# RobotLocomotion/pytorch-dense-correspondence

Measured on NVIDIA H100. Metric: image-pairs/s (640x480, D=3) fwd+loss+bwd, higher is better.
Workload: dtype f32 (bf16x3 split on the wgmma tensor cores, fp32 accumulate)

## Files before the change

pytorch-dense-correspondence_b200/csrc/conv_tc.cu:

```cuda
#include <cuda.h>
#include <algorithm>
#include <cstring>
#include <functional>
#include <mutex>
#include <unordered_map>

#include "conv.cuh"
#include "conv_tc.cuh"

namespace ddn {

constexpr int TC_BLOCK_K = 64;
constexpr int TC_CONSUMERS = 256;
constexpr int TC_THREADS = TC_CONSUMERS + 32;
constexpr int TC_PRODUCER_WARP = TC_CONSUMERS / 32;
constexpr int TC_WIDE_THREADS = TC_CONSUMERS + 128;
constexpr int TC_A_BYTES = 128 * TC_BLOCK_K * 2;

__device__ __forceinline__ uint32_t smem_u32(const void* p) { return (uint32_t)__cvta_generic_to_shared(p); }

__device__ __forceinline__ void mbar_init(uint32_t bar, uint32_t count) {
  asm volatile("mbarrier.init.shared::cta.b64 [%0], %1;" ::"r"(bar), "r"(count));
}
__device__ __forceinline__ void mbar_expect_tx(uint32_t bar, uint32_t bytes) {
// ... 110 lines not shown
  if (NPROD == 3) {
    Wgmma<N>::template mma<TRANS>(d, a_hi, b_lo, accumulate);
    Wgmma<N>::template mma<TRANS>(d, a_lo, b_hi, 1);
    Wgmma<N>::template mma<TRANS>(d, a_hi, b_hi, 1);
  } else {
    Wgmma<N>::template mma<TRANS>(d, a_hi, b_hi, accumulate);
  }
}
template <int N, int TRANS, int NPROD>
__device__ __forceinline__ void mma_k16_x(float (&d)[N / 2], float (&x)[N / 2], uint64_t a_hi, uint64_t a_lo, uint64_t b_hi, uint64_t b_lo,
                                          int accumulate) {
  if (NPROD == 3) {
    Wgmma<N>::template mma<TRANS>(x, a_hi, b_lo, accumulate);
    Wgmma<N>::template mma<TRANS>(x, a_lo, b_hi, 1);
  }
  Wgmma<N>::template mma<TRANS>(d, a_hi, b_hi, accumulate);
}
template <int K>
__device__ __forceinline__ void add_cross(float (&d)[K], const float (&x)[K]) {
#pragma unroll
  for (int i = 0; i < K; ++i) d[i] += x[i];
}
template <int N, int K>
__device__ __forceinline__ float (&acc_cols(float (&d)[K]))[N / 2] {
  static_assert(N / 2 <= K, "accumulator too narrow");
  return *reinterpret_cast<float(*)[N / 2]>(&d[0]);
}

constexpr int EPI_ROWS = 4;
constexpr int EPI_STRIDE = 40;
constexpr int EPI_WARP_FLOATS = 16 * EPI_STRIDE;

template <int K>
__device__ __forceinline__ void stage_write(const float (&acc)[K], int c, float* st, int lane) {
  const int r = lane >> 2, q = (lane & 3) * 2;
#pragma unroll
  for (int jj = 0; jj < 4; ++jj) {
    const int j = 4 * c + jj;
    *reinterpret_cast<float2*>(st + r * EPI_STRIDE + 8 * jj + q) = make_float2(acc[4 * j], acc[4 * j + 1]);
    *reinterpret_cast<float2*>(st + (r + 8) * EPI_STRIDE + 8 * jj + q) = make_float2(acc[4 * j + 2], acc[4 * j + 3]);
  }
  __syncwarp();
}

template <int K>
__device__ __forceinline__ void stage_chunk(const float (&acc)[K], int c, float* st, int lane, float4 (&v)[EPI_ROWS]) {
  stage_write(acc, c, st, lane);
  const int ga = lane >> 3, gb = lane & 7;
#pragma unroll
  for (int i = 0; i < EPI_ROWS; ++i) v[i] = *reinterpret_cast<const float4*>(st + (EPI_ROWS * ga + i) * EPI_STRIDE + 4 * gb);
  __syncwarp();
}

__device__ __forceinline__ uint32_t pack_bf16x2(__nv_bfloat16 a, __nv_bfloat16 b) {
  return (uint32_t)__bfloat16_as_ushort(a) | ((uint32_t)__bfloat16_as_ushort(b) << 16);
}

struct TcEpilogueParams {
  float* out;
  const float* addend;
  int imgs_per_group;
  BnFwdFinal fin;
  TcBwdStats bst;
  const float* ep_scale; const float* ep_shift; int ep_relu;
  __nv_bfloat16* out_hi; __nv_bfloat16* out_lo;
};

__device__ __forceinline__ void conv_epilogue_rows(const TcEpilogueParams& p, const float4 (&v)[EPI_ROWS], size_t off, size_t rs, int n_ok, int ch,
                                                   int C, int grp, float4& s1, float4& s2) {
  float4 adv[EPI_ROWS];
#pragma unroll
  for (int i = 0; i < EPI_ROWS; ++i)
    adv[i] = (p.addend && i < n_ok) ? __ldg(reinterpret_cast<const float4*>(p.addend + off + i * rs)) : make_float4(0.f, 0.f, 0.f, 0.f);
  if (p.ep_scale) {
    const float4 sc = __ldg(reinterpret_cast<const float4*>(p.ep_scale + ch));
    const float4 sh = __ldg(reinterpret_cast<const float4*>(p.ep_shift + ch));
#pragma unroll
    for (int i = 0; i < EPI_ROWS; ++i) {
      float4 f = make_float4(fmaf(v[i].x, sc.x, sh.x) + adv[i].x, fmaf(v[i].y, sc.y, sh.y) + adv[i].y,
                             fmaf(v[i].z, sc.z, sh.z) + adv[i].z, fmaf(v[i].w, sc.w, sh.w) + adv[i].w);
      if (p.ep_relu) { f.x = fmaxf(f.x, 0.f); f.y = fmaxf(f.y, 0.f); f.z = fmaxf(f.z, 0.f); f.w = fmaxf(f.w, 0.f); }
      if (i < n_ok) {
        if (p.out) *reinterpret_cast<float4*>(p.out + off + i * rs) = f;
        if (p.out_hi) {
          const __nv_bfloat16 h0 = __float2bfloat16_rn(f.x), h1 = __float2bfloat16_rn(f.y), h2 = __float2bfloat16_rn(f.z), h3 = __float2bfloat16_rn(f.w);
          *reinterpret_cast<uint2*>(p.out_hi + off + i * rs) = make_uint2(pack_bf16x2(h0, h1), pack_bf16x2(h2, h3));
          if (p.out_lo)
            *reinterpret_cast<uint2*>(p.out_lo + off + i * rs) =
                make_uint2(pack_bf16x2(__float2bfloat16_rn(f.x - __bfloat162float(h0)), __float2bfloat16_rn(f.y - __bfloat162float(h1))),
                           pack_bf16x2(__float2bfloat16_rn(f.z - __bfloat162float(h2)), __float2bfloat16_rn(f.w - __bfloat162float(h3))));
        }
      }
    }
  } else if (p.bst.fin.a.acc) {
    float4 rw[EPI_ROWS];
    uint2 yh[EPI_ROWS];
#pragma unroll
    for (int i = 0; i < EPI_ROWS; ++i) {
      rw[i] = i < n_ok ? __ldg(reinterpret_cast<const float4*>(p.bst.raw + off + i * rs)) : make_float4(0.f, 0.f, 0.f, 0.f);
      if (p.bst.y_hi) yh[i] = i < n_ok ? __ldg(reinterpret_cast<const uint2*>(p.bst.y_hi + off + i * rs)) : make_uint2(0u, 0u);
    }
    const float4 mu = __ldg(reinterpret_cast<const float4*>(p.bst.mean + (size_t)grp * C + ch));
    const float4 is = __ldg(reinterpret_cast<const float4*>(p.bst.invstd + (size_t)grp * C + ch));
    float4 scl = make_float4(0.f, 0.f, 0.f, 0.f), be = scl;
    if (!p.bst.y_hi && p.bst.relu) {
      const float4 gm = __ldg(reinterpret_cast<const float4*>(p.bst.gamma + ch));
      be = __ldg(reinterpret_cast<const float4*>(p.bst.beta + ch));
      scl = make_float4(gm.x * is.x, gm.y * is.y, gm.z * is.z, gm.w * is.w);
    }
#pragma unroll
    for (int i = 0; i < EPI_ROWS; ++i) {
      float4 g = make_float4(v[i].x + adv[i].x, v[i].y + adv[i].y, v[i].z + adv[i].z, v[i].w + adv[i].w);
      if (i < n_ok) *reinterpret_cast<float4*>(p.out + off + i * rs) = g;
      else g = make_float4(0.f, 0.f, 0.f, 0.f);
      if (p.bst.y_hi) {
        const uint2 hh = yh[i];
        if ((hh.x & 0x8000u) || !(hh.x & 0x7fffu)) g.x = 0.f;
        if ((hh.x & 0x80000000u) || !(hh.x & 0x7fff0000u)) g.y = 0.f;
        if ((hh.y & 0x8000u) || !(hh.y & 0x7fffu)) g.z = 0.f;
        if ((hh.y & 0x80000000u) || !(hh.y & 0x7fff0000u)) g.w = 0.f;
      } else if (p.bst.relu) {
        if (!(fmaf(rw[i].x - mu.x, scl.x, be.x) > 0.f)) g.x = 0.f;
        if (!(fmaf(rw[i].y - mu.y, scl.y, be.y) > 0.f)) g.y = 0.f;
        if (!(fmaf(rw[i].z - mu.z, scl.z, be.z) > 0.f)) g.z = 0.f;
        if (!(fmaf(rw[i].w - mu.w, scl.w, be.w) > 0.f)) g.w = 0.f;
      }
      s1.x += g.x; s1.y += g.y; s1.z += g.z; s1.w += g.w;
      s2.x = fmaf(g.x, (rw[i].x - mu.x) * is.x, s2.x); s2.y = fmaf(g.y, (rw[i].y - mu.y) * is.y, s2.y);
      s2.z = fmaf(g.z, (rw[i].z - mu.z) * is.z, s2.z); s2.w = fmaf(g.w, (rw[i].w - mu.w) * is.w, s2.w);
    }
  } else {
#pragma unroll
    for (int i = 0; i < EPI_ROWS; ++i) {
      const float4 raw = i < n_ok ? v[i] : make_float4(0.f, 0.f, 0.f, 0.f);
      if (i < n_ok)
        *reinterpret_cast<float4*>(p.out + off + i * rs) = make_float4(raw.x + adv[i].x, raw.y + adv[i].y, raw.z + adv[i].z, raw.w + adv[i].w);
      s1.x += raw.x; s1.y += raw.y; s1.z += raw.z; s1.w += raw.w;
      s2.x = fmaf(raw.x, raw.x, s2.x); s2.y = fmaf(raw.y, raw.y, s2.y); s2.z = fmaf(raw.z, raw.z, s2.z); s2.w = fmaf(raw.w, raw.w, s2.w);
    }
  }
}

__device__ __forceinline__ void colsum_lane_groups(float4& s1, float4& s2) {
#pragma unroll
  for (int off = 8; off < 32; off <<= 1) {
    s1.x += __shfl_xor_sync(0xffffffffu, s1.x, off); s1.y += __shfl_xor_sync(0xffffffffu, s1.y, off);
    s1.z += __shfl_xor_sync(0xffffffffu, s1.z, off); s1.w += __shfl_xor_sync(0xffffffffu, s1.w, off);
    s2.x += __shfl_xor_sync(0xffffffffu, s2.x, off); s2.y += __shfl_xor_sync(0xffffffffu, s2.y, off);
    s2.z += __shfl_xor_sync(0xffffffffu, s2.z, off); s2.w += __shfl_xor_sync(0xffffffffu, s2.w, off);
  }
}

__device__ __forceinline__ void named_barrier(int id, int threads) { asm volatile("bar.sync %0, %1;" ::"r"(id), "r"(threads) : "memory"); }
// ... 30 lines not shown
    const int j = idx - p.full_items;
    tile = p.full_items + j / p.tail_split;
    piece = j - (j / p.tail_split) * p.tail_split;
    width = block_n / p.tail_split;
  }
  TcItem it;
  it.sp = tile / p.n_co;
  it.co0 = (tile - it.sp * p.n_co) * block_n + piece * width;
  it.width = width;
  return it;
}
struct TcSub { int n, h0, w0; bool valid; };
__device__ __forceinline__ TcSub tc_sub(const TcConvParams& p, int st) {
  TcSub s;
  s.valid = st < p.n_sub;
  const int tw = st % p.tiles_w; const int t = st / p.tiles_w;
  const int th = t % p.tiles_h;
  s.n = s.valid ? t / p.tiles_h : p.N;
  s.h0 = th * TC_SUB_H; s.w0 = tw * TC_SUB_W;
  return s;
}

template <int W, int BLOCK_N, int NPROD, int STAGES, int TRANS = 0>
__device__ __forceinline__ void conv_tc_mainloop(float (&acc)[W / 2], float (&accx)[W / 2], int num_kb, uint32_t& g, const uint64_t* full_bar,
                                                 const uint64_t* empty_bar, const uint8_t* smem, int wg, int lane) {
  constexpr int NSPLIT = NPROD == 3 ? 2 : 1;
  constexpr int A_BYTES = 128 * TC_BLOCK_K * 2;
  constexpr int B_BYTES = BLOCK_N * TC_BLOCK_K * 2;
  constexpr int STAGE_BYTES = NSPLIT * (A_BYTES + B_BYTES);
  constexpr uint32_t LBO = TRANS ? TC_SUB_BYTES : 16;
  constexpr int K_STEP = TRANS ? 16 * 128 : 32;
  for (int kb = 0; kb < num_kb; ++kb, ++g) {
    const int s = g % STAGES;
    mbar_wait(smem_u32(&full_bar[s]), (g / STAGES) & 1);
    wgmma_fence();
    const uint32_t stg = smem_u32(smem + (size_t)s * STAGE_BYTES);
    const uint64_t a_hi = gmma_desc(stg + wg * TC_SUB_BYTES, LBO, 1024), a_lo = gmma_desc(stg + A_BYTES + wg * TC_SUB_BYTES, LBO, 1024);
    const uint64_t b_hi = gmma_desc(stg + NSPLIT * A_BYTES, LBO, 1024), b_lo = gmma_desc(stg + 2 * A_BYTES + B_BYTES, LBO, 1024);
#pragma unroll
    for (int k = 0; k < TC_BLOCK_K / 16; ++k) {
      const uint64_t adv = (uint64_t)((k * K_STEP) >> 4);
      mma_k16_x<W, TRANS, NPROD>(acc, accx, a_hi + adv, a_lo + adv, b_hi + adv, b_lo + adv, (kb | k) != 0);
    }
    wgmma_commit();
    wgmma_wait<1>();
    if (kb > 0 && lane == 0) mbar_arrive(smem_u32(&empty_bar[(g - 1) % STAGES]));
  }
  wgmma_wait<0>();
  fence_acc(acc);
  if (NPROD == 3) { fence_acc(accx); add_cross(acc, accx); }
  if (lane == 0) mbar_arrive(smem_u32(&empty_bar[(g - 1) % STAGES]));
}

template <int BLOCK_N, int NPROD>
__global__ void __launch_bounds__(TC_WIDE_THREADS, 1)
conv_tc_kernel(const __grid_constant__ CUtensorMap tm_a_hi, const __grid_constant__ CUtensorMap tm_a_lo,
               const __grid_constant__ CUtensorMap tm_b_hi, const __grid_constant__ CUtensorMap tm_b_lo,
               const __grid_constant__ CUtensorMap tm_bt_hi, const __grid_constant__ CUtensorMap tm_bt_lo,
               const TcConvParams p) {
  constexpr int NSPLIT = NPROD == 3 ? 2 : 1;
  constexpr int A_BYTES = 128 * TC_BLOCK_K * 2;
  constexpr int B_BYTES = BLOCK_N * TC_BLOCK_K * 2;
  constexpr int STAGE_BYTES = NSPLIT * (A_BYTES + B_BYTES);
  constexpr int STAGES = (192 * 1024) / STAGE_BYTES >= 8 ? 8 : (192 * 1024) / STAGE_BYTES;
  static_assert(STAGES >= 2, "pipeline needs at least two stages");

  extern __shared__ __align__(1024) uint8_t smem_raw[];
  uint8_t* smem = reinterpret_cast<uint8_t*>((reinterpret_cast<uintptr_t>(smem_raw) + 1023) & ~uintptr_t(1023));
  __shared__ __align__(8) uint64_t full_bar[STAGES];
  __shared__ __align__(8) uint64_t empty_bar[STAGES];
  __shared__ int s_last;
  __shared__ __align__(16) float s_stage[TC_CONSUMERS / 32][EPI_WARP_FLOATS];
  __shared__ __align__(16) float s_part[2][2][4][BLOCK_N];

  pdl_trigger();
  const int warp = __shfl_sync(0xffffffffu, threadIdx.x >> 5, 0), lane = threadIdx.x & 31;
  const int cin_chunks = p.Cin / TC_BLOCK_K;
  const int num_kb = p.taps_w * p.taps_w * cin_chunks;
  const int half = p.taps_w >> 1;

  if (threadIdx.x == 0) {
    for (int s = 0; s < STAGES; ++s) { mbar_init(smem_u32(&full_bar[s]), 1); mbar_init(smem_u32(&empty_bar[s]), TC_CONSUMERS / 32); }
    fence_barrier_init();
    tma_prefetch_desc(&tm_a_hi); tma_prefetch_desc(&tm_b_hi); tma_prefetch_desc(&tm_bt_hi);
    if (NSPLIT == 2) { tma_prefetch_desc(&tm_a_lo); tma_prefetch_desc(&tm_b_lo); tma_prefetch_desc(&tm_bt_lo); }
  }
  __syncthreads();
  pdl_wait();

  if (warp >= TC_PRODUCER_WARP) {
    setmaxnreg_dec<40>();
    if (warp == TC_PRODUCER_WARP && lane == 0) {
      uint32_t g = 0;
      for (int idx = blockIdx.x; idx < p.total_items; idx += gridDim.x) {
        const TcItem it = tc_item(p, idx, BLOCK_N);
        const bool tail = it.width != BLOCK_N;
        const uint32_t stage_tx = (uint32_t)(NSPLIT * (A_BYTES + it.width * TC_BLOCK_K * 2));
        const CUtensorMap* mb_hi = tail ? &tm_bt_hi : &tm_b_hi;
        const CUtensorMap* mb_lo = tail ? &tm_bt_lo : &tm_b_lo;
        const TcSub s0 = tc_sub(p, it.sp * 2), s1 = tc_sub(p, it.sp * 2 + 1);
        for (int kb = 0; kb < num_kb; ++kb, ++g) {
          const int s = g % STAGES;
          mbar_wait(smem_u32(&empty_bar[s]), ((g / STAGES) & 1) ^ 1);
          const int tap = kb / cin_chunks, cc = kb - tap * cin_chunks;
          const int r = tap / p.taps_w, sx = tap - r * p.taps_w;
          const int dh = (r - half) * p.dil, dw = (sx - half) * p.dil;
          uint8_t* stg = smem + (size_t)s * STAGE_BYTES;
          const uint32_t bar = smem_u32(&full_bar[s]);
          mbar_expect_tx(bar, stage_tx);
          tma_load_4d(smem_u32(stg), &tm_a_hi, bar, cc * TC_BLOCK_K, s0.w0 * p.stride + dw, s0.h0 * p.stride + dh, s0.n);
          tma_load_4d(smem_u32(stg + TC_SUB_BYTES), &tm_a_hi, bar, cc * TC_BLOCK_K, s1.w0 * p.stride + dw, s1.h0 * p.stride + dh, s1.n);
          tma_load_2d(smem_u32(stg + NSPLIT * A_BYTES), mb_hi, bar, kb * TC_BLOCK_K, it.co0);
          if (NSPLIT == 2) {
            tma_load_4d(smem_u32(stg + A_BYTES), &tm_a_lo, bar, cc * TC_BLOCK_K, s0.w0 * p.stride + dw, s0.h0 * p.stride + dh, s0.n);
            tma_load_4d(smem_u32(stg + A_BYTES + TC_SUB_BYTES), &tm_a_lo, bar, cc * TC_BLOCK_K, s1.w0 * p.stride + dw, s1.h0 * p.stride + dh, s1.n);
            tma_load_2d(smem_u32(stg + 2 * A_BYTES + B_BYTES), mb_lo, bar, kb * TC_BLOCK_K, it.co0);
          }
        }
      }
    }
  } else {
    setmaxnreg_inc<232>();
    const int wg = warp >> 2, w = warp & 3, e = threadIdx.x & 127;
    const int ga = lane >> 3, gb = lane & 7;
    const bool stats = p.epi.fin.a.acc != nullptr;
    const bool bstats = p.epi.bst.fin.a.acc != nullptr;
    double* const sum_acc = bstats ? p.epi.bst.fin.a.acc : p.epi.fin.a.acc;
    float* const st = s_stage[warp];
    float acc[BLOCK_N / 2], accx[BLOCK_N / 2];
    uint32_t g = 0;
    for (int idx = blockIdx.x; idx < p.total_items; idx += gridDim.x) {
      const TcItem it = tc_item(p, idx, BLOCK_N);
      if (it.width == BLOCK_N)
        conv_tc_mainloop<BLOCK_N, BLOCK_N, NPROD, STAGES>(acc, accx, num_kb, g, full_bar, empty_bar, smem, wg, lane);
      else if (BLOCK_N > 64 && it.width == 64)
        conv_tc_mainloop<64, BLOCK_N, NPROD, STAGES>(acc_cols<64>(acc), acc_cols<64>(accx), num_kb, g, full_bar, empty_bar, smem, wg, lane);
      else
        conv_tc_mainloop<32, BLOCK_N, NPROD, STAGES>(acc_cols<32>(acc), acc_cols<32>(accx), num_kb, g, full_bar, empty_bar, smem, wg, lane);

      const TcSub sb = tc_sub(p, it.sp * 2 + wg);
      const int h = sb.h0 + w, w4 = sb.w0 + EPI_ROWS * ga;
      const int n_ok = (sb.valid && h < p.H) ? min(EPI_ROWS, p.W - w4) : 0;
      const size_t pix = ((size_t)(n_ok > 0 ? sb.n : 0) * p.H + (n_ok > 0 ? h : 0)) * p.W + (n_ok > 0 ? w4 : 0);
      const size_t cbase = pix * p.Cout + it.co0 + gb * 4;
      const int grp = sb.valid ? sb.n / p.epi.imgs_per_group : 0;
#pragma unroll
      for (int c = 0; c < BLOCK_N / 32; ++c) {
        if (c < (it.width >> 5)) {
          float4 v[EPI_ROWS];
          stage_chunk(acc, c, st, lane, v);
          float4 s1 = make_float4(0.f, 0.f, 0.f, 0.f), s2 = s1;
          conv_epilogue_rows(p.epi, v, cbase + c * 32, (size_t)p.Cout, n_ok, it.co0 + c * 32 + gb * 4, p.Cout, grp, s1, s2);
          if (stats || bstats) {
            colsum_lane_groups(s1, s2);
            if (ga == 0) {
              *reinterpret_cast<float4*>(&s_part[wg][0][w][c * 32 + gb * 4]) = s1;
              *reinterpret_cast<float4*>(&s_part[wg][1][w][c * 32 + gb * 4]) = s2;
            }
          }
        }
      }
      if (stats || bstats) {
        named_barrier(1 + wg, 128);
        if (sb.valid)
          for (int col = e; col < it.width; col += 128) {
#pragma unroll
            for (int k = 0; k < 2; ++k) {
              const float sum = s_part[wg][k][0][col] + s_part[wg][k][1][col] + s_part[wg][k][2][col] + s_part[wg][k][3][col];
              red_add_f64(sum_acc + (size_t)(grp * 2 + k) * p.Cout + it.co0 + col, (double)sum);
            }
          }
        named_barrier(1 + wg, 128);
      }
    }
    conv_epilogue_finalize(p.epi, p.Cout, &s_last, 3);
  }
}

struct TcHaloParams {
  TcEpilogueParams epi;
  int N, H, W;
  int tiles_h, tiles_w, n_tiles;
};
constexpr int HALO_TH = 8, HALO_TW = 16;
constexpr int HALO_BH = HALO_TH + 2, HALO_BW = HALO_TW + 2;
constexpr int HALO_BOX_BYTES = HALO_BH * HALO_BW * 128;
constexpr int HALO_SLOT = ((HALO_BOX_BYTES + 1023) / 1024) * 1024;
constexpr int HALO_B_TAP = 64 * 128;
constexpr int HALO_B_PLANE = 9 * HALO_B_TAP;
__host__ __device__ constexpr int halo_slots(int nprod) { return nprod == 3 ? 2 : 3; }

template <int NPROD>
__global__ void __launch_bounds__(TC_THREADS, 1)
conv64_halo_kernel(const __grid_constant__ CUtensorMap tm_a_hi, const __grid_constant__ CUtensorMap tm_a_lo,
                   const __grid_constant__ CUtensorMap tm_b_hi, const __grid_constant__ CUtensorMap tm_b_lo, const TcHaloParams p) {
  constexpr int NSPLIT = NPROD == 3 ? 2 : 1;
  constexpr int SLOTS = halo_slots(NPROD);
  extern __shared__ __align__(1024) uint8_t smem_raw[];
  uint8_t* smem = reinterpret_cast<uint8_t*>((reinterpret_cast<uintptr_t>(smem_raw) + 1023) & ~uintptr_t(1023));
  uint8_t* smem_b = smem;
  uint8_t* smem_a = smem + NSPLIT * HALO_B_PLANE;
  __shared__ __align__(8) uint64_t full_bar[SLOTS], empty_bar[SLOTS], b_full;
  __shared__ int s_last;
  __shared__ __align__(16) float s_stage[TC_CONSUMERS / 32][EPI_WARP_FLOATS];
  __shared__ __align__(16) float s_part[2][8][64];
// ... 619 lines not shown
    for (int v : {k.d0, k.d1, k.d2, k.d3, k.b0, k.b1, k.b2, k.sample}) h = h * 1000003u ^ (size_t)v;
    return h;
  }
};
static std::unordered_map<MapKey, CUtensorMap, MapKeyHash> g_maps;
static std::mutex g_maps_mu;

static int make_act_map(CUtensorMap* m, const void* base, int N, int H, int W, int C, int sample = 1) {
  const MapKey key = {base, C, W, H, N, TC_BLOCK_K, TC_SUB_W, TC_SUB_H, sample};
  {
    std::lock_guard<std::mutex> lk(g_maps_mu);
    auto it = g_maps.find(key);
    if (it != g_maps.end()) { *m = it->second; return 0; }
  }
  EncodeTiledFn enc = get_encode_fn();
  if (!enc) { set_error("cuTensorMapEncodeTiled is unavailable (driver too old?)"); return DDN_EUNSUPPORTED; }
  cuuint64_t dims[4] = {(cuuint64_t)C, (cuuint64_t)W, (cuuint64_t)H, (cuuint64_t)N};
  cuuint64_t strides[3] = {(cuuint64_t)C * 2, (cuuint64_t)W * C * 2, (cuuint64_t)H * W * C * 2};
  cuuint32_t box[4] = {(cuuint32_t)TC_BLOCK_K, (cuuint32_t)(TC_SUB_W * sample), (cuuint32_t)(TC_SUB_H * sample), 1};
  cuuint32_t es[4] = {1, (cuuint32_t)sample, (cuuint32_t)sample, 1};
  CUresult r = enc(m, CU_TENSOR_MAP_DATA_TYPE_BFLOAT16, 4, const_cast<void*>(base), dims, strides, box, es,
                   CU_TENSOR_MAP_INTERLEAVE_NONE, CU_TENSOR_MAP_SWIZZLE_128B, CU_TENSOR_MAP_L2_PROMOTION_L2_128B,
                   CU_TENSOR_MAP_FLOAT_OOB_FILL_NONE);
  if (r != CUDA_SUCCESS) { set_error("cuTensorMapEncodeTiled(activations) failed: %d", (int)r); return DDN_EINVAL; }
  std::lock_guard<std::mutex> lk(g_maps_mu);
  if (g_maps.size() > 8192) g_maps.clear();
  g_maps[key] = *m;
  return 0;
}
static int make_act_map_hw(CUtensorMap* m, const void* base, int N, int H, int W, int C, int box_h, int box_w) {
  const MapKey key = {base, C, H, W, N, TC_BLOCK_K, box_h, box_w, -2};
  {
    std::lock_guard<std::mutex> lk(g_maps_mu);
    auto it = g_maps.find(key);
    if (it != g_maps.end()) { *m = it->second; return 0; }
  }
  EncodeTiledFn enc = get_encode_fn();
  if (!enc) { set_error("cuTensorMapEncodeTiled is unavailable (driver too old?)"); return DDN_EUNSUPPORTED; }
  cuuint64_t dims[4] = {(cuuint64_t)C, (cuuint64_t)H, (cuuint64_t)W, (cuuint64_t)N};
  cuuint64_t strides[3] = {(cuuint64_t)W * C * 2, (cuuint64_t)C * 2, (cuuint64_t)H * W * C * 2};
  cuuint32_t box[4] = {(cuuint32_t)TC_BLOCK_K, (cuuint32_t)box_h, (cuuint32_t)box_w, 1};
  cuuint32_t es[4] = {1, 1, 1, 1};
  CUresult r = enc(m, CU_TENSOR_MAP_DATA_TYPE_BFLOAT16, 4, const_cast<void*>(base), dims, strides, box, es,
                   CU_TENSOR_MAP_INTERLEAVE_NONE, CU_TENSOR_MAP_SWIZZLE_128B, CU_TENSOR_MAP_L2_PROMOTION_L2_128B,
                   CU_TENSOR_MAP_FLOAT_OOB_FILL_NONE);
  if (r != CUDA_SUCCESS) { set_error("cuTensorMapEncodeTiled(halo activations) failed: %d", (int)r); return DDN_EINVAL; }
  std::lock_guard<std::mutex> lk(g_maps_mu);
  if (g_maps.size() > 8192) g_maps.clear();
  g_maps[key] = *m;
  return 0;
}
static int make_act_map_halo(CUtensorMap* m, const void* base, int N, int H, int W, int C) {
  return make_act_map_hw(m, base, N, H, W, C, HALO_BH, HALO_BW);
}
static int make_weight_map(CUtensorMap* m, const void* base, int rows, int K, int box_rows) {
  const MapKey key = {base, K, rows, 0, 0, TC_BLOCK_K, box_rows, 0, -1};
  {
    std::lock_guard<std::mutex> lk(g_maps_mu);
    auto it = g_maps.find(key);
    if (it != g_maps.end()) { *m = it->second; return 0; }
  }
  EncodeTiledFn enc = get_encode_fn();
  if (!enc) { set_error("cuTensorMapEncodeTiled is unavailable (driver too old?)"); return DDN_EUNSUPPORTED; }
  cuuint64_t dims[2] = {(cuuint64_t)K, (cuuint64_t)rows};
  cuuint64_t strides[1] = {(cuuint64_t)K * 2};
  cuuint32_t box[2] = {(cuuint32_t)TC_BLOCK_K, (cuuint32_t)box_rows};
  cuuint32_t es[2] = {1, 1};
  CUresult r = enc(m, CU_TENSOR_MAP_DATA_TYPE_BFLOAT16, 2, const_cast<void*>(base), dims, strides, box, es,
                   CU_TENSOR_MAP_INTERLEAVE_NONE, CU_TENSOR_MAP_SWIZZLE_128B, CU_TENSOR_MAP_L2_PROMOTION_L2_256B,
                   CU_TENSOR_MAP_FLOAT_OOB_FILL_NONE);
  if (r != CUDA_SUCCESS) { set_error("cuTensorMapEncodeTiled(weights) failed: %d", (int)r); return DDN_EINVAL; }
  std::lock_guard<std::mutex> lk(g_maps_mu);
  if (g_maps.size() > 8192) g_maps.clear();
  g_maps[key] = *m;
  return 0;
}

template <int BN, int NPROD>
static int launch_wgrad_tc(const CUtensorMap& dy_hi, const CUtensorMap& dy_lo, const CUtensorMap& x_hi, const CUtensorMap& x_lo,
                           const TcWgradParams& p, int workers, cudaStream_t st) {
  constexpr int NSPLIT = NPROD == 3 ? 2 : 1;
  constexpr int STAGE_BYTES = NSPLIT * (TC_A_BYTES + BN * TC_BLOCK_K * 2);
  constexpr int STAGES = (192 * 1024) / STAGE_BYTES >= 8 ? 8 : (192 * 1024) / STAGE_BYTES;
  const size_t smem = (size_t)STAGES * STAGE_BYTES + 1024;
  static bool configured = false;
  if (!configured) {
    DDN_CUDA(cudaFuncSetAttribute(wgrad_tc_kernel<BN, NPROD>, cudaFuncAttributeMaxDynamicSharedMemorySize, (int)smem));
    configured = true;
  }
  DDN_LAUNCH((wgrad_tc_kernel<BN, NPROD>), workers, TC_WIDE_THREADS, smem, st, dy_hi, dy_lo, x_hi, x_lo, p);
  return 0;
}

static int tc_wgrad_chunks(int tiles, int total_kb, int workers) {
  const double even = (double)tiles * total_kb / workers;
  const int max_s = std::max(1, total_kb / 4);
  int best = 1;
  double best_span = 1e300;
  for (int s = 1; s <= max_s; ++s) {
    const double span = (double)ceil_div((int64_t)s * tiles, workers) * (double)ceil_div(total_kb, s);
    if (span <= 1.02 * even) return s;
    if (span < best_span) { best_span = span; best = s; }
  }
  return best;
}

// ... 59 lines not shown
    DDN_LAUNCH(unpack_wgrad_tc_kernel, blocks, 256, 0, st, dwp, dw, Cout, Cin, taps);
  }
  return 0;
}

int tc_unpack_wgrads(const TcUnpackEntry* entries, int n, const double* dwp_base, float* grads_base, cudaStream_t st) {
  for (int i0 = 0; i0 < n; i0 += TC_UNPACK_MAX) {
    TcUnpackTable t; t.n = std::min(TC_UNPACK_MAX, n - i0);
    int64_t biggest = 0;
    for (int i = 0; i < t.n; ++i) { t.e[i] = entries[i0 + i]; biggest = std::max<int64_t>(biggest, (int64_t)t.e[i].Cout * t.e[i].Cin * t.e[i].taps); }
    dim3 grid((unsigned)std::min<int64_t>(ceil_div(biggest, 256 * 4), 1024), (unsigned)t.n);
    DDN_LAUNCH(unpack_wgrad_batched_kernel, grid, 256, 0, st, dwp_base, grads_base, t);
  }
  return 0;
}

bool tc_conv_supported(int Cin, int Cout, int k, int stride, int pad, int dil, int H, int W) {
  if (Cin % 64 || Cout % 64) return false;
  if (stride == 2) { if (dil != 1 || (H & 1) || (W & 1)) return false; }
  else if (stride != 1) return false;
  if (k == 3) return pad == dil;
  if (k == 1) return pad == 0;
  return false;
}

static const size_t kMaxWeightElems = (size_t)9 * 512 * 512;
size_t tc_max_weight_elems() { return kMaxWeightElems; }
size_t tc_weight_ws_bytes() { return 2 * align_up(kMaxWeightElems * 2, 1024) + 2048; }

int tc_split(const float* x, __nv_bfloat16* hi, __nv_bfloat16* lo, int64_t n, int precision, cudaStream_t st) {
  DDN_CHECK_ARG(n % 4 == 0, "split: element count must be a multiple of 4");
  int64_t n4 = n / 4;
  int blocks = (int)std::min<int64_t>(ceil_div(n4, 256), (int64_t)num_sms() * 8);
  DDN_LAUNCH(split_bf16_kernel, blocks, 256, 0, st, x, hi, lo, n4, precision == DDN_PRECISION_BF16X3 ? 1 : 0);
  return 0;
}

int tc_upsample_zero_split(const float* dy, __nv_bfloat16* hi, __nv_bfloat16* lo, int N, int Ho, int Wo, int C, int precision,
                           cudaStream_t st) {
  int64_t total = (int64_t)N * Ho * Wo * (C / 4);
  int blocks = (int)std::min<int64_t>(ceil_div(total, 256), (int64_t)num_sms() * 8);
  DDN_LAUNCH(upsample_zero_split_kernel, blocks, 256, 0, st, dy, hi, lo, N, Ho, Wo, C, precision == DDN_PRECISION_BF16X3 ? 1 : 0);
  return 0;
}

int tc_stem_patches(const float* x_nchw, __nv_bfloat16* hi, __nv_bfloat16* lo, int N, int H, int W, int precision, cudaStream_t st) {
  const int H1 = (H - 1) / 2 + 1, W1 = (W - 1) / 2 + 1;
  DDN_CHECK_ARG(N <= 65535 && H1 <= 65535, "stem: batch / height too large for the launch grid");
  dim3 grid((unsigned)ceil_div(W1, STEM_TW), (unsigned)H1, (unsigned)N);
  DDN_LAUNCH(stem_patch_split_kernel, grid, 256, 0, st, x_nchw, hi, lo, N, H, W, H1, W1, precision == DDN_PRECISION_BF16X3 ? 1 : 0);
  return 0;
}

template <int BLOCK_N, int NPROD>
static int launch_conv_tc(const CUtensorMap& a_hi, const CUtensorMap& a_lo, const CUtensorMap& b_hi, const CUtensorMap& b_lo,
                          const CUtensorMap& bt_hi, const CUtensorMap& bt_lo, const TcConvParams& p, int workers, cudaStream_t st) {
  constexpr int NSPLIT = NPROD == 3 ? 2 : 1;
  constexpr int STAGE_BYTES = NSPLIT * (128 * TC_BLOCK_K * 2 + BLOCK_N * TC_BLOCK_K * 2);
  constexpr int STAGES = (192 * 1024) / STAGE_BYTES >= 8 ? 8 : (192 * 1024) / STAGE_BYTES;
  const size_t smem = (size_t)STAGES * STAGE_BYTES + 1024;
  static bool configured = false;
  if (!configured) {
    DDN_CUDA(cudaFuncSetAttribute(conv_tc_kernel<BLOCK_N, NPROD>, cudaFuncAttributeMaxDynamicSharedMemorySize, (int)smem));
    configured = true;
  }
  DDN_LAUNCH((conv_tc_kernel<BLOCK_N, NPROD>), workers, TC_WIDE_THREADS, smem, st, a_hi, a_lo, b_hi, b_lo, bt_hi, bt_lo, p);
  return 0;
}

template <int NPROD>
static int launch_conv64_halo(const CUtensorMap& a_hi, const CUtensorMap& a_lo, const CUtensorMap& b_hi, const CUtensorMap& b_lo,
                              const TcHaloParams& p, cudaStream_t st) {
  constexpr int NSPLIT = NPROD == 3 ? 2 : 1;
  const size_t smem = (size_t)NSPLIT * HALO_B_PLANE + (size_t)halo_slots(NPROD) * HALO_SLOT + 1024;
  static bool configured = false;
  if (!configured) {
    DDN_CUDA(cudaFuncSetAttribute(conv64_halo_kernel<NPROD>, cudaFuncAttributeMaxDynamicSharedMemorySize, (int)smem));
    configured = true;
  }
  const int grid = std::min(p.n_tiles, tc_worker_sms());
  DDN_LAUNCH((conv64_halo_kernel<NPROD>), grid, TC_THREADS, smem, st, a_hi, a_lo, b_hi, b_lo, p);
  return 0;
}

static int tc_epilogue_request(TcEpilogueParams* e, float* out, const float* addend, const BnFwdFinal* stats, const TcBwdStats* bst,
                               const TcFoldedEpilogue* ep, int N, int gout, int dgrad, int want_lo) {
  memset(e, 0, sizeof(*e));
  e->out = out; e->addend = addend; e->imgs_per_group = N;
  if (stats) {
    DDN_CHECK_ARG(!dgrad && !ep && stats->G >= 1 && stats->G <= BN_MAX_GROUPS && N % stats->G == 0 && stats->C == gout,
                  "bad BatchNorm statistics request");
    e->fin = *stats;
    e->imgs_per_group = N / stats->G;
  }
  if (bst) {
    DDN_CHECK_ARG(dgrad && !ep && !stats && bst->raw && bst->mean && bst->invstd && bst->fin.a.acc && bst->fin.G >= 1 &&
                  bst->fin.G <= BN_MAX_GROUPS && N % bst->fin.G == 0 && bst->fin.C == gout && (bst->y_hi || !bst->relu || (bst->gamma && bst->beta)),
                  "bad BatchNorm backward-statistics request");
    e->bst = *bst;
    e->imgs_per_group = N / bst->fin.G;
  }
  if (ep) {
    DDN_CHECK_ARG(!dgrad && !stats && !bst && ep->scale && ep->shift && (out || ep->out_hi), "folded epilogue: forward only, needs scale/shift and an output");
    e->ep_scale = ep->scale; e->ep_shift = ep->shift; e->ep_relu = ep->relu; e->out_hi = ep->out_hi; e->out_lo = want_lo ? ep->out_lo : nullptr;
  } else {
    DDN_CHECK_ARG(out != nullptr, "conv output pointer is null");
  }
  return 0;
}

int tc_conv_planes(TcPlanes in, const float* w_oihw, const TcPlanes* wpk, float* out, const float* addend, const BnFwdFinal* stats,
                   int N, int H, int W, int Cin, int Cout, int k, int stride, int dil, int dgrad, int precision,
                   void* wws, size_t wws_bytes, cudaStream_t st, const TcFoldedEpilogue* ep, const TcBwdStats* bst) {
  DDN_CHECK_ARG(stride == 1 || !dgrad, "the strided data gradient goes through zero-inserted planes (stride 1 here)");
  const int Ho = H / stride, Wo = W / stride;
  const double fl = 2.0 * N * Ho * Wo * (double)Cout * k * k * Cin;
  const int gin = dgrad ? Cout : Cin, gout = dgrad ? Cin : Cout;
  const int want_lo = precision == DDN_PRECISION_BF16X3;
  TcEpilogueParams epi;
// ... 1 lines not shown
  const __nv_bfloat16* b_hi; const __nv_bfloat16* b_lo;
  if (wpk) {
    b_hi = wpk->hi; b_lo = wpk->lo;
  } else {
    const size_t wel = (size_t)Cout * Cin * k * k;
    const size_t w_b = align_up(kMaxWeightElems * 2, 1024);
    DDN_CHECK_ARG(wws != nullptr && wel <= kMaxWeightElems, "tc weight staging missing or weight tensor too large");
    char* base = reinterpret_cast<char*>(align_up(reinterpret_cast<uintptr_t>(wws), 1024));
    if ((size_t)(base - (char*)wws) + 2 * w_b > wws_bytes) { set_error("tensor-core weight staging too small"); return DDN_EWORKSPACE; }
    __nv_bfloat16* ph = (__nv_bfloat16*)base; __nv_bfloat16* pl = (__nv_bfloat16*)(base + w_b);
    int wblocks = (int)std::min<int64_t>(ceil_div((int64_t)wel, 256), 4096);
    DDN_LAUNCH(pack_weights_tc_kernel, wblocks, 256, 0, st, w_oihw, ph, pl, Cout, Cin, k, dgrad, want_lo);
    b_hi = ph; b_lo = pl;
  }
  if (k == 3 && gin == 64 && gout == 64 && stride == 1 && dil == 1 && Ho % HALO_TH == 0 && Wo % HALO_TW == 0) {
    TcHaloParams hp;
    memset(&hp, 0, sizeof(hp));
    hp.epi = epi; hp.N = N; hp.H = Ho; hp.W = Wo;
    hp.tiles_h = Ho / HALO_TH; hp.tiles_w = Wo / HALO_TW; hp.n_tiles = N * hp.tiles_h * hp.tiles_w;
    CUtensorMap ma_hi, ma_lo, mb_hi, mb_lo;
    DDN_TRY(make_act_map_halo(&ma_hi, in.hi, N, H, W, 64));
    DDN_TRY(make_act_map_halo(&ma_lo, want_lo ? in.lo : in.hi, N, H, W, 64));
    DDN_TRY(make_weight_map(&mb_hi, b_hi, 64, 9 * 64, 64));
    DDN_TRY(make_weight_map(&mb_lo, want_lo ? b_lo : b_hi, 64, 9 * 64, 64));
    ProfScope ps(dgrad ? PROF_CONV_DGRAD_TC : PROF_CONV_FWD_TC, fl, st);
    return want_lo ? launch_conv64_halo<3>(ma_hi, ma_lo, mb_hi, mb_lo, hp, st) : launch_conv64_halo<1>(ma_hi, ma_lo, mb_hi, mb_lo, hp, st);
  }
  const int block_n = gout % 128 == 0 ? 128 : 64;
  TcConvParams p;
  memset(&p, 0, sizeof(p));
  p.epi = epi; p.N = N; p.H = Ho; p.W = Wo; p.Cin = gin; p.Cout = gout; p.taps_w = k; p.dil = dil;
  p.stride = stride;
  p.tiles_h = (int)ceil_div(Ho, TC_SUB_H); p.tiles_w = (int)ceil_div(Wo, TC_SUB_W);
  p.n_sub = N * p.tiles_h * p.tiles_w;
  p.n_co = gout / block_n;
  const int tiles = (int)ceil_div(p.n_sub, 2) * p.n_co;
  const int workers_max = tc_worker_sms();
  const int rem = tiles % workers_max;
  int split = 1;
  if (rem)
    while (split * 2 <= 8 && block_n / (split * 2) >= 32 && rem * split * 2 <= workers_max) split *= 2;
  p.full_items = tiles - rem; p.tail_split = split; p.total_items = p.full_items + rem * split;
  if (split == 1) { p.full_items = tiles; p.total_items = tiles; }
  const int workers = std::min(p.total_items, workers_max);
  const int b_rows = block_n;
  const int bt_rows = b_rows / split;
  CUtensorMap ma_hi, ma_lo, mb_hi, mb_lo, mt_hi, mt_lo;
  DDN_TRY(make_act_map(&ma_hi, in.hi, N, H, W, gin, stride));
  DDN_TRY(make_act_map(&ma_lo, want_lo ? in.lo : in.hi, N, H, W, gin, stride));
  DDN_TRY(make_weight_map(&mb_hi, b_hi, gout, k * k * gin, b_rows));
  DDN_TRY(make_weight_map(&mb_lo, want_lo ? b_lo : b_hi, gout, k * k * gin, b_rows));
  DDN_TRY(make_weight_map(&mt_hi, b_hi, gout, k * k * gin, bt_rows));
  DDN_TRY(make_weight_map(&mt_lo, want_lo ? b_lo : b_hi, gout, k * k * gin, bt_rows));
  ProfScope ps(dgrad ? PROF_CONV_DGRAD_TC : PROF_CONV_FWD_TC, fl, st);
#define CONV_TC(BN)                                                                                                           \
  (want_lo ? launch_conv_tc<BN, 3>(ma_hi, ma_lo, mb_hi, mb_lo, mt_hi, mt_lo, p, workers, st)                                   \
           : launch_conv_tc<BN, 1>(ma_hi, ma_lo, mb_hi, mb_lo, mt_hi, mt_lo, p, workers, st))
  if (block_n == 128) return CONV_TC(128);
  return CONV_TC(64);
#undef CONV_TC
}

int tc_dgrad_strided(const float* dy_f32, TcPlanes up, const float* w_oihw, const TcPlanes* w_packed, float* dx, const float* addend,
                     int N, int H, int W, int Cin, int Cout, int k, int precision, void* wws, size_t wws_bytes, cudaStream_t st,
                     const TcBwdStats* bst) {
  DDN_TRY(tc_upsample_zero_split(dy_f32, const_cast<__nv_bfloat16*>(up.hi), const_cast<__nv_bfloat16*>(up.lo), N, H / 2, W / 2, Cout,
                                 precision, st));
  return tc_conv_planes(up, w_oihw, w_packed, dx, addend, nullptr, N, H, W, Cin, Cout, k, 1, 1, 1, precision, wws, wws_bytes, st, nullptr, bst);
}

int tc_stem_pack_weights(const float* w_conv1, __nv_bfloat16* hi, __nv_bfloat16* lo, int precision, cudaStream_t st) {
  DDN_LAUNCH(stem_pack_weights_kernel, (64 * 192 + 255) / 256, 256, 0, st, w_conv1, hi, lo, precision == DDN_PRECISION_BF16X3 ? 1 : 0);
  return 0;
}
int tc_stem_forward(TcPlanes patches, const float* w_conv1, const TcPlanes* w_packed, float* raw, const BnFwdFinal* stats, int N, int H1,
                    int W1, int precision, void* wws, size_t wws_bytes, cudaStream_t st) {
  TcPlanes wpk;
  if (w_packed) wpk = *w_packed;
  else {
    char* base = reinterpret_cast<char*>(align_up(reinterpret_cast<uintptr_t>(wws), 1024));
    DDN_CHECK_ARG((size_t)(base - (char*)wws) + 2 * 64 * 192 * 2 + 1024 <= wws_bytes, "weight staging too small");
    __nv_bfloat16* ph = (__nv_bfloat16*)base; __nv_bfloat16* pl = (__nv_bfloat16*)(base + align_up((size_t)64 * 192 * 2, 1024));
    DDN_TRY(tc_stem_pack_weights(w_conv1, ph, pl, precision, st));
    wpk.hi = ph; wpk.lo = pl;
  }
  return tc_conv_planes(patches, nullptr, &wpk, raw, nullptr, stats, N, H1, W1, 192, 64, 1, 1, 1, 0, precision, wws, wws_bytes, st);
}

int tc_stem_wgrad(TcPlanes patches, TcPlanes dy, float* dw_conv1, int N, int H1, int W1, int precision, double* scratch, cudaStream_t st) {
  if (!dw_conv1) return tc_wgrad_planes(patches, dy, nullptr, N, H1, W1, 192, 64, 1, 1, 1, precision, scratch, st);
  double* dwp = scratch; float* dwk = reinterpret_cast<float*>(scratch + 64 * 192);
  DDN_TRY(tc_wgrad_planes(patches, dy, dwk, N, H1, W1, 192, 64, 1, 1, 1, precision, dwp, st));
  DDN_LAUNCH(stem_unpack_wgrad_kernel, (64 * 147 + 255) / 256, 256, 0, st, dwk, dw_conv1);
  return 0;
}

int tc_pack_all(const float* params, int64_t n_params, char* cache, const TcPackEntry* entries, int n, unsigned long long* fp_new,
                unsigned long long* fp_old, int force, int precision, cudaStream_t st) {
  DDN_CHECK_ARG(n >= 1, "empty pack table");
  DDN_LAUNCH(param_fingerprint_kernel, num_sms() * 2, 256, 0, st, reinterpret_cast<const uint32_t*>(params), n_params, fp_new);
  for (int i0 = 0; i0 < n; i0 += TC_PACK_MAX) {
    TcPackTable t; t.n = std::min(TC_PACK_MAX, n - i0);
    for (int i = 0; i < t.n; ++i) t.e[i] = entries[i0 + i];
    dim3 grid(32, (unsigned)t.n);
    DDN_LAUNCH(pack_all_kernel, grid, 256, 0, st, params, cache, t, fp_new, fp_old, force, precision == DDN_PRECISION_BF16X3 ? 1 : 0);
  }
  DDN_LAUNCH(commit_fingerprint_kernel, 1, 32, 0, st, fp_new, fp_old);
  return 0;
}

size_t tc_workspace_bytes(size_t max_act_elems) { return tc_weight_ws_bytes() + 6 * align_up(max_act_elems * 2, 1024) + 4096; }

// ... 45 lines not shown
```

Baseline: 142.3.

## Prefetch backward-stat epilogue operands via TMA through the mainloop pipeline stages

For the backward BN-stats epilogue variant, the producer warp now issues TMA loads of the raw pre-activation, addend and bf16 y_hi tiles into the pipeline's shared-memory stages after the K loop. Consumers wait on the full barriers and read these operands from shared memory instead of doing strided __ldg global loads. This overlaps epilogue operand fetch with compute and uses bulk transfers, at the cost of extra tensor maps, a templated kernel variant, and more complex barrier phase bookkeeping. The y_hi row-ordering flip logic is a correctness risk.

```diff
diff --git a/pytorch-dense-correspondence_b200/csrc/conv_tc.cu b/pytorch-dense-correspondence_b200/csrc/conv_tc.cu
--- a/pytorch-dense-correspondence_b200/csrc/conv_tc.cu
+++ b/pytorch-dense-correspondence_b200/csrc/conv_tc.cu
@@ -186,6 +186,12 @@
   __syncwarp();
 }
 
+constexpr int EPI_BOX_F32 = 64 * 32 * 4;
+constexpr int EPI_BOX_BF16 = 64 * 32 * 2;
+constexpr int EPI_SUB_BYTES = 2 * EPI_BOX_F32 + EPI_BOX_BF16;
+
+struct EpiSlot { const float* raw; const float* add; const uint2* yh; int flip; };
+
 __device__ __forceinline__ uint32_t pack_bf16x2(__nv_bfloat16 a, __nv_bfloat16 b) {
   return (uint32_t)__bfloat16_as_ushort(a) | ((uint32_t)__bfloat16_as_ushort(b) << 16);
 }
@@ -200,13 +206,16 @@
   __nv_bfloat16* out_hi; __nv_bfloat16* out_lo;
 };
 
+template <bool BST = false>
 __device__ __forceinline__ void conv_epilogue_rows(const TcEpilogueParams& p, const float4 (&v)[EPI_ROWS], size_t off, size_t rs, int n_ok, int ch,
-                                                   int C, int grp, float4& s1, float4& s2) {
+                                                   int C, int grp, float4& s1, float4& s2, const EpiSlot* es = nullptr) {
   float4 adv[EPI_ROWS];
 #pragma unroll
   for (int i = 0; i < EPI_ROWS; ++i)
-    adv[i] = (p.addend && i < n_ok) ? __ldg(reinterpret_cast<const float4*>(p.addend + off + i * rs)) : make_float4(0.f, 0.f, 0.f, 0.f);
-  if (p.ep_scale) {
+    adv[i] = !p.addend ? make_float4(0.f, 0.f, 0.f, 0.f)
+             : es      ? *reinterpret_cast<const float4*>(es->add + i * 32)
+             : i < n_ok ? __ldg(reinterpret_cast<const float4*>(p.addend + off + i * rs)) : make_float4(0.f, 0.f, 0.f, 0.f);
+  if (!BST && p.ep_scale) {
     const float4 sc = __ldg(reinterpret_cast<const float4*>(p.ep_scale + ch));
     const float4 sh = __ldg(reinterpret_cast<const float4*>(p.ep_shift + ch));
 #pragma unroll
@@ -226,13 +235,25 @@
         }
       }
     }
-  } else if (p.bst.fin.a.acc) {
+  } else if (BST || p.bst.fin.a.acc) {
     float4 rw[EPI_ROWS];
     uint2 yh[EPI_ROWS];
-#pragma unroll
-    for (int i = 0; i < EPI_ROWS; ++i) {
-      rw[i] = i < n_ok ? __ldg(reinterpret_cast<const float4*>(p.bst.raw + off + i * rs)) : make_float4(0.f, 0.f, 0.f, 0.f);
-      if (p.bst.y_hi) yh[i] = i < n_ok ? __ldg(reinterpret_cast<const uint2*>(p.bst.y_hi + off + i * rs)) : make_uint2(0u, 0u);
+    if (es) {
+#pragma unroll
+      for (int i = 0; i < EPI_ROWS; ++i) {
+        rw[i] = *reinterpret_cast<const float4*>(es->raw + i * 32);
+        if (p.bst.y_hi) yh[i] = es->yh[(i ^ es->flip) * 8];
+      }
+      if (p.bst.y_hi && es->flip) {
+        uint2 t = yh[0]; yh[0] = yh[1]; yh[1] = t;
+        t = yh[2]; yh[2] = yh[3]; yh[3] = t;
+      }
+    } else {
+#pragma unroll
+      for (int i = 0; i < EPI_ROWS; ++i) {
+        rw[i] = i < n_ok ? __ldg(reinterpret_cast<const float4*>(p.bst.raw + off + i * rs)) : make_float4(0.f, 0.f, 0.f, 0.f);
+        if (p.bst.y_hi) yh[i] = i < n_ok ? __ldg(reinterpret_cast<const uint2*>(p.bst.y_hi + off + i * rs)) : make_uint2(0u, 0u);
+      }
     }
     const float4 mu = __ldg(reinterpret_cast<const float4*>(p.bst.mean + (size_t)grp * C + ch));
     const float4 is = __ldg(reinterpret_cast<const float4*>(p.bst.invstd + (size_t)grp * C + ch));
@@ -369,11 +390,13 @@
   if (lane == 0) mbar_arrive(smem_u32(&empty_bar[(g - 1) % STAGES]));
 }
 
-template <int BLOCK_N, int NPROD>
+template <int BLOCK_N, int NPROD, bool BST>
 __global__ void __launch_bounds__(TC_WIDE_THREADS, 1)
 conv_tc_kernel(const __grid_constant__ CUtensorMap tm_a_hi, const __grid_constant__ CUtensorMap tm_a_lo,
                const __grid_constant__ CUtensorMap tm_b_hi, const __grid_constant__ CUtensorMap tm_b_lo,
                const __grid_constant__ CUtensorMap tm_bt_hi, const __grid_constant__ CUtensorMap tm_bt_lo,
+               const __grid_constant__ CUtensorMap tm_raw, const __grid_constant__ CUtensorMap tm_add,
+               const __grid_constant__ CUtensorMap tm_yh,
                const TcConvParams p) {
   constexpr int NSPLIT = NPROD == 3 ? 2 : 1;
   constexpr int A_BYTES = 128 * TC_BLOCK_K * 2;
@@ -381,6 +404,9 @@
   constexpr int STAGE_BYTES = NSPLIT * (A_BYTES + B_BYTES);
   constexpr int STAGES = (192 * 1024) / STAGE_BYTES >= 8 ? 8 : (192 * 1024) / STAGE_BYTES;
   static_assert(STAGES >= 2, "pipeline needs at least two stages");
+  constexpr int EPI_PER_SLOT = STAGE_BYTES >= 2 * EPI_SUB_BYTES ? 2 : 1;
+  constexpr int EPI_SLOTS = 2 / EPI_PER_SLOT;
+  static_assert(STAGE_BYTES >= EPI_SUB_BYTES, "a stage must hold one sub-tile's epilogue operands");
 
   extern __shared__ __align__(1024) uint8_t smem_raw[];
   uint8_t* smem = reinterpret_cast<uint8_t*>((reinterpret_cast<uintptr_t>(smem_raw) + 1023) & ~uintptr_t(1023));
@@ -401,6 +427,11 @@
     fence_barrier_init();
     tma_prefetch_desc(&tm_a_hi); tma_prefetch_desc(&tm_b_hi); tma_prefetch_desc(&tm_bt_hi);
     if (NSPLIT == 2) { tma_prefetch_desc(&tm_a_lo); tma_prefetch_desc(&tm_b_lo); tma_prefetch_desc(&tm_bt_lo); }
+    if (BST) {
+      tma_prefetch_desc(&tm_raw);
+      if (p.epi.addend) tma_prefetch_desc(&tm_add);
+      if (p.epi.bst.y_hi) tma_prefetch_desc(&tm_yh);
+    }
   }
   __syncthreads();
   pdl_wait();
@@ -434,14 +465,35 @@
             tma_load_2d(smem_u32(stg + 2 * A_BYTES + B_BYTES), mb_lo, bar, kb * TC_BLOCK_K, it.co0);
           }
         }
+        if (BST) {
+          const uint32_t sub_tx = (uint32_t)(EPI_BOX_F32 + (p.epi.addend ? EPI_BOX_F32 : 0) + (p.epi.bst.y_hi ? EPI_BOX_BF16 : 0));
+          for (int c = 0; c < (it.width >> 5); ++c) {
+            for (int j = 0; j < EPI_SLOTS; ++j, ++g) {
+              const int s = g % STAGES;
+              mbar_wait(smem_u32(&empty_bar[s]), ((g / STAGES) & 1) ^ 1);
+              uint8_t* stg = smem + (size_t)s * STAGE_BYTES;
+              const uint32_t bar = smem_u32(&full_bar[s]);
+              mbar_expect_tx(bar, EPI_PER_SLOT * sub_tx);
+              for (int q = 0; q < EPI_PER_SLOT; ++q) {
+                const TcSub& sb = (j * EPI_PER_SLOT + q) ? s1 : s0;
+                const uint32_t dst = smem_u32(stg + q * EPI_SUB_BYTES);
+                const int ch = it.co0 + c * 32;
+                tma_load_4d(dst, &tm_raw, bar, ch, sb.w0, sb.h0, sb.n);
+                if (p.epi.addend) tma_load_4d(dst + EPI_BOX_F32, &tm_add, bar, ch, sb.w0, sb.h0, sb.n);
+                if (p.epi.bst.y_hi) tma_load_4d(dst + 2 * EPI_BOX_F32, &tm_yh, bar, ch, sb.w0, sb.h0, sb.n);
+              }
+            }
+          }
+        }
       }
     }
   } else {
     setmaxnreg_inc<232>();
     const int wg = warp >> 2, w = warp & 3, e = threadIdx.x & 127;
     const int ga = lane >> 3, gb = lane & 7;
-    const bool stats = p.epi.fin.a.acc != nullptr;
-    const bool bstats = p.epi.bst.fin.a.acc != nullptr;
+    const int epx = (w * TC_SUB_W + EPI_ROWS * ga) * 32 + gb * 4;
+    const bool stats = !BST && p.epi.fin.a.acc != nullptr;
+    const bool bstats = BST;
     double* const sum_acc = bstats ? p.epi.bst.fin.a.acc : p.epi.fin.a.acc;
     float* const st = s_stage[warp];
     float acc[BLOCK_N / 2], accx[BLOCK_N / 2];
@@ -467,7 +519,20 @@
           float4 v[EPI_ROWS];
           stage_chunk(acc, c, st, lane, v);
           float4 s1 = make_float4(0.f, 0.f, 0.f, 0.f), s2 = s1;
-          conv_epilogue_rows(p.epi, v, cbase + c * 32, (size_t)p.Cout, n_ok, it.co0 + c * 32 + gb * 4, p.Cout, grp, s1, s2);
+          if (bstats) {
+            for (int j = 0; j < EPI_SLOTS; ++j) mbar_wait(smem_u32(&full_bar[(g + j) % STAGES]), ((g + j) / STAGES) & 1);
+            const uint8_t* sub = smem + (size_t)((g + wg / EPI_PER_SLOT) % STAGES) * STAGE_BYTES + (wg % EPI_PER_SLOT) * EPI_SUB_BYTES;
+            const float* raw = reinterpret_cast<const float*>(sub) + epx;
+            const EpiSlot es = {raw, raw + EPI_BOX_F32 / 4,
+                                reinterpret_cast<const uint2*>(reinterpret_cast<const __nv_bfloat16*>(sub + 2 * EPI_BOX_F32) + epx), ga & 1};
+            conv_epilogue_rows<true>(p.epi, v, cbase + c * 32, (size_t)p.Cout, n_ok, it.co0 + c * 32 + gb * 4, p.Cout, grp, s1, s2, &es);
+            __syncwarp();
+            if (lane == 0)
+              for (int j = 0; j < EPI_SLOTS; ++j) mbar_arrive(smem_u32(&empty_bar[(g + j) % STAGES]));
+            g += EPI_SLOTS;
+          } else {
+            conv_epilogue_rows(p.epi, v, cbase + c * 32, (size_t)p.Cout, n_ok, it.co0 + c * 32 + gb * 4, p.Cout, grp, s1, s2);
+          }
           if (stats || bstats) {
             colsum_lane_groups(s1, s2);
             if (ga == 0) {
@@ -1193,6 +1258,28 @@
 }
 static int make_act_map_halo(CUtensorMap* m, const void* base, int N, int H, int W, int C) {
   return make_act_map_hw(m, base, N, H, W, C, HALO_BH, HALO_BW);
+}
+static int make_epi_map(CUtensorMap* m, const void* base, int esize, int N, int H, int W, int C) {
+  const MapKey key = {base, C, W, H, N, 32, TC_SUB_W, TC_SUB_H, -esize};
+  {
+    std::lock_guard<std::mutex> lk(g_maps_mu);
+    auto it = g_maps.find(key);
+    if (it != g_maps.end()) { *m = it->second; return 0; }
+  }
+  EncodeTiledFn enc = get_encode_fn();
+  if (!enc) { set_error("cuTensorMapEncodeTiled is unavailable (driver too old?)"); return DDN_EUNSUPPORTED; }
+  cuuint64_t dims[4] = {(cuuint64_t)C, (cuuint64_t)W, (cuuint64_t)H, (cuuint64_t)N};
+  cuuint64_t strides[3] = {(cuuint64_t)C * esize, (cuuint64_t)W * C * esize, (cuuint64_t)H * W * C * esize};
+  cuuint32_t box[4] = {32, (cuuint32_t)TC_SUB_W, (cuuint32_t)TC_SUB_H, 1};
+  cuuint32_t es[4] = {1, 1, 1, 1};
+  CUresult r = enc(m, esize == 4 ? CU_TENSOR_MAP_DATA_TYPE_FLOAT32 : CU_TENSOR_MAP_DATA_TYPE_BFLOAT16, 4, const_cast<void*>(base), dims, strides,
+                   box, es, CU_TENSOR_MAP_INTERLEAVE_NONE, CU_TENSOR_MAP_SWIZZLE_NONE, CU_TENSOR_MAP_L2_PROMOTION_L2_128B,
+                   CU_TENSOR_MAP_FLOAT_OOB_FILL_NONE);
+  if (r != CUDA_SUCCESS) { set_error("cuTensorMapEncodeTiled(epilogue operands) failed: %d", (int)r); return DDN_EINVAL; }
+  std::lock_guard<std::mutex> lk(g_maps_mu);
+  if (g_maps.size() > 8192) g_maps.clear();
+  g_maps[key] = *m;
+  return 0;
 }
 static int make_weight_map(CUtensorMap* m, const void* base, int rows, int K, int box_rows) {
   const MapKey key = {base, K, rows, 0, 0, TC_BLOCK_K, box_rows, 0, -1};
@@ -1358,19 +1445,20 @@
   return 0;
 }
 
-template <int BLOCK_N, int NPROD>
+template <int BLOCK_N, int NPROD, bool BST>
 static int launch_conv_tc(const CUtensorMap& a_hi, const CUtensorMap& a_lo, const CUtensorMap& b_hi, const CUtensorMap& b_lo,
-                          const CUtensorMap& bt_hi, const CUtensorMap& bt_lo, const TcConvParams& p, int workers, cudaStream_t st) {
+                          const CUtensorMap& bt_hi, const CUtensorMap& bt_lo, const CUtensorMap (&epi)[3], const TcConvParams& p, int workers,
+                          cudaStream_t st) {
   constexpr int NSPLIT = NPROD == 3 ? 2 : 1;
   constexpr int STAGE_BYTES = NSPLIT * (128 * TC_BLOCK_K * 2 + BLOCK_N * TC_BLOCK_K * 2);
   constexpr int STAGES = (192 * 1024) / STAGE_BYTES >= 8 ? 8 : (192 * 1024) / STAGE_BYTES;
   const size_t smem = (size_t)STAGES * STAGE_BYTES + 1024;
   static bool configured = false;
   if (!configured) {
-    DDN_CUDA(cudaFuncSetAttribute(conv_tc_kernel<BLOCK_N, NPROD>, cudaFuncAttributeMaxDynamicSharedMemorySize, (int)smem));
+    DDN_CUDA(cudaFuncSetAttribute(conv_tc_kernel<BLOCK_N, NPROD, BST>, cudaFuncAttributeMaxDynamicSharedMemorySize, (int)smem));
     configured = true;
   }
-  DDN_LAUNCH((conv_tc_kernel<BLOCK_N, NPROD>), workers, TC_WIDE_THREADS, smem, st, a_hi, a_lo, b_hi, b_lo, bt_hi, bt_lo, p);
+  DDN_LAUNCH((conv_tc_kernel<BLOCK_N, NPROD, BST>), workers, TC_WIDE_THREADS, smem, st, a_hi, a_lo, b_hi, b_lo, bt_hi, bt_lo, epi[0], epi[1], epi[2], p);
   return 0;
 }
 
@@ -1478,12 +1566,19 @@
   DDN_TRY(make_weight_map(&mb_lo, want_lo ? b_lo : b_hi, gout, k * k * gin, b_rows));
   DDN_TRY(make_weight_map(&mt_hi, b_hi, gout, k * k * gin, bt_rows));
   DDN_TRY(make_weight_map(&mt_lo, want_lo ? b_lo : b_hi, gout, k * k * gin, bt_rows));
+  CUtensorMap me[3];
+  memset(me, 0, sizeof(me));
+  if (bst) {
+    DDN_TRY(make_epi_map(&me[0], bst->raw, 4, N, Ho, Wo, gout));
+    if (addend) DDN_TRY(make_epi_map(&me[1], addend, 4, N, Ho, Wo, gout));
+    if (bst->y_hi) DDN_TRY(make_epi_map(&me[2], bst->y_hi, 2, N, Ho, Wo, gout));
+  }
   ProfScope ps(dgrad ? PROF_CONV_DGRAD_TC : PROF_CONV_FWD_TC, fl, st);
-#define CONV_TC(BN)                                                                                                           \
-  (want_lo ? launch_conv_tc<BN, 3>(ma_hi, ma_lo, mb_hi, mb_lo, mt_hi, mt_lo, p, workers, st)                                   \
-           : launch_conv_tc<BN, 1>(ma_hi, ma_lo, mb_hi, mb_lo, mt_hi, mt_lo, p, workers, st))
-  if (block_n == 128) return CONV_TC(128);
-  return CONV_TC(64);
+#define CONV_TC(BN, BST)                                                                                                      \
+  (want_lo ? launch_conv_tc<BN, 3, BST>(ma_hi, ma_lo, mb_hi, mb_lo, mt_hi, mt_lo, me, p, workers, st)                          \
+           : launch_conv_tc<BN, 1, BST>(ma_hi, ma_lo, mb_hi, mb_lo, mt_hi, mt_lo, me, p, workers, st))
+  if (block_n == 128) return bst ? CONV_TC(128, true) : CONV_TC(128, false);
+  return bst ? CONV_TC(64, true) : CONV_TC(64, false);
 #undef CONV_TC
 }
 
```

Measured after the change: 143.9 (median of 6 runs). 1.1% higher.
